# pigBond/olympics-mujoco

Hardware: AMD Instinct MI355X
Metric: env-steps/sec, 4096 UnitreeH1.walk envs per GPU, obs+reward+done+ctrl HIP kernel (higher is better)
Workload: dtype f64; 1 GPU; UnitreeH1.walk config-2: fused K1+K5 over one [T,N] block per step; T=400, envs_per_gpu=4096, launch_regime=[T,N] block per launch, io=qpos/qvel f64 + action f32 in; obs/reward/ctrl f32 + absorbing u8 out, parallelism=env-sharded x1, no data-path collective

## Files before the change

olympics-mujoco_amd/csrc/k1_il_step.hip:

```cpp
#include <cstdlib>

#include "oly_common.h"

namespace {

constexpr int THREADS = 256;
typedef unsigned int u32x4 __attribute__((ext_vector_type(4)));

template <int NQ, int NV, int NGRF, int NACT, int NU, int NOBS>
struct StaticDims {
  static constexpr int nq = NQ, nv = NV, n_grf = NGRF, n_act = NACT, nu = NU, n_obs = NOBS;
  static constexpr bool is_static = true;
  static constexpr int n_obs_ct = NOBS;
  template <int ROWS, int TH>
  static constexpr int max_chunks() {
    return (ROWS * (NQ + NV + NGRF) / 2 + ROWS * NACT / 4 + TH - 1) / TH;
  }
  __device__ explicit StaticDims(const IlDev*) {}
};
struct DynDims {
  int nq, nv, n_grf, n_act, nu, n_obs;
  static constexpr bool is_static = false;
  static constexpr int n_obs_ct = 1;
  template <int ROWS, int TH>
  static constexpr int max_chunks() { return 1; }
  __device__ explicit DynDims(const IlDev* m)
      : nq(m->nq), nv(m->nv), n_grf(m->n_grf), n_act(m->n_act), nu(m->nu), n_obs(m->n_obs) {}
};

struct IlArgs {
  const IlDev* md;
  long R;
  int N;
  const double* qpos;
  const double* qvel;
  const float* action;
  const double* grf;
  const double* prev_in;
  double* prev_out;
  void* obs;
  float* reward;
  uint8_t* absorbing;
  uint8_t* fall_code;
  void* ctrl;
  int fast;
  long tile0;
};

template <int ROWS, class D>
struct Carve {
  int q, v, g, a, tab_off, tab_str, tab_csrc, tab_act, total;
  __host__ __device__ Carve(int nq, int nv, int n_grf, int n_act, int nu, int n_obs) {
    auto al = [](int x) { return (x + 15) & ~15; };
    q = 0;
    v = q + ROWS * nq * 8;
    g = v + ROWS * nv * 8;
    a = al(g + ROWS * n_grf * 8);
    tab_off = al(a + ROWS * n_act * 4);
    tab_str = al(tab_off + n_obs * 4);
    tab_csrc = al(tab_str + n_obs * 4);
    tab_act = al(tab_csrc + nu * 4);
    total = al(tab_act + 4 * nu * 8);
  }
};

#ifndef OLY_K1_NT
#define OLY_K1_NT 1
#endif
typedef float f32x4 __attribute__((ext_vector_type(4)));
typedef double f64x2 __attribute__((ext_vector_type(2)));
__device__ __forceinline__ u32x4 ld16(const u32x4* p) {
  return (OLY_K1_NT & 1) ? __builtin_nontemporal_load(p) : *p;
}
__device__ __forceinline__ void st16(f32x4* p, f32x4 v) {
  if (OLY_K1_NT & 2) __builtin_nontemporal_store(v, p); else *p = v;
}
__device__ __forceinline__ void st16(f64x2* p, f64x2 v) {
  if (OLY_K1_NT & 2) __builtin_nontemporal_store(v, p); else *p = v;
}

#ifndef OLY_K1_ABLATE
#define OLY_K1_ABLATE 0
#endif

// ... 481 lines not shown
#pragma unroll
      for (int k = FAST_FALL - 1; k >= 0; --k)
        if (fv[k] < f_lo[k] || fv[k] > f_hi[k]) code = (unsigned)(k + 1);
      const unsigned ab = (code != 0 && use_abs) ? 1u : 0u;
      if (rt == OLY_REWARD_NONE) {
        p.reward[gr] = 0.0f;
      } else {
        if (gr < p.N) p.reward[gr] = rew_f(p.prev_in[gr]);
        if (gr + p.N < p.R)
          p.reward[gr + p.N] = rew_f(x);
        else
          p.prev_out[gr - (p.R - p.N)] = x;
      }
      unsigned a4 = 0, c4 = 0;
#pragma unroll
      for (int k = 0; k < 4; ++k) {
        const int srcl = (lane & 15) * 4 + k;
        a4 |= (unsigned)__shfl((int)ab, srcl, 64) << (8 * k);
        c4 |= (unsigned)__shfl((int)code, srcl, 64) << (8 * k);
      }
      if (lane < 16) {
        const long q4 = (row0 + (r - lane)) / 4 + lane;
        reinterpret_cast<unsigned*>(p.absorbing)[q4] = a4;
        if (p.fall_code) reinterpret_cast<unsigned*>(p.fall_code)[q4] = c4;
      }
    }

    {
      double v[NIT][OW];
#pragma unroll
      for (int it = 0; it < NIT; ++it)
#pragma unroll
        for (int k = 0; k < OW; ++k) {
          v[it][k] = sq[e_off[it][k]];
          if (NG > 0 && ((e_grf >> (it * OW + k)) & 1u)) v[it][k] = v[it][k] / 1000.0;
        }
#pragma unroll
      for (int it = 0; it < NIT; ++it) {
        const int i = tid + it * THREADS;
        if (it * THREADS + THREADS <= NOV || i < NOV) {
          if (OBS64) {
            f64x2 o;
            o.x = v[it][0]; o.y = v[it][OW - 1];
            st16(reinterpret_cast<f64x2*>(static_cast<double*>(p.obs) + row0 * NO) + i, o);
          } else {
            f32x4 o;
            o.x = (float)v[it][0]; o.y = (float)v[it][1 % OW];
            o.z = (float)v[it][2 % OW]; o.w = (float)v[it][3 % OW];
            st16(reinterpret_cast<f32x4*>(static_cast<float*>(p.obs) + row0 * NO) + i, o);
          }
        }
      }
    }

    if (with_ctrl) {
#pragma unroll
      for (int it = 0; it < NCI; ++it) {
        const int i = tid + it * THREADS;
        if (it * THREADS + THREADS <= NCV || i < NCV) {
          double u[CW];
#pragma unroll
          for (int q = 0; q < CW; ++q) {
            const int ai = c_aidx[it][q], j = c_j[it][q];
            const double a = (double)sa[ai < 0 ? 0 : ai];
            double x = a * t_act[NU + j] + t_act[j];
            const double lo = t_act[2 * NU + j], hi = t_act[3 * NU + j];
            if (x < lo) x = lo;
            if (x > hi) x = hi;
            u[q] = ai < 0 ? 0.0 : x;
          }
          if (CTRL64) {
            f64x2 o;
            o.x = u[0]; o.y = u[CW - 1];
            st16(reinterpret_cast<f64x2*>(static_cast<double*>(p.ctrl) + row0 * NU) + i, o);
          } else {
            f32x4 o;
            o.x = (float)u[0]; o.y = (float)u[1 % CW]; o.z = (float)u[2 % CW]; o.w = (float)u[3 % CW];
            st16(reinterpret_cast<f32x4*>(static_cast<float*>(p.ctrl) + row0 * NU) + i, o);
          }
        }
      }
    }
    __syncthreads();
  }
}

template <bool CTRL64>
__global__ __launch_bounds__(THREADS) void il_ctrl_kernel(const IlDev* __restrict__ md, long total,
                                                          const float* __restrict__ action,
                                                          void* __restrict__ ctrl) {
  const int nu = md->nu, n_act = md->n_act;
  const long stride = (long)gridDim.x * THREADS;
  for (long e = (long)blockIdx.x * THREADS + threadIdx.x; e < total; e += stride) {
    const long r = e / nu;
    const int j = (int)(e - r * nu);
    const int k = md->ctrl_src[j];
    double u = 0.0;
    if (k >= 0) {
      u = (double)action[r * n_act + k] * md->act_delta[k] + md->act_mean[k];
      if (u < md->ctrl_lo[k]) u = md->ctrl_lo[k];
      if (u > md->ctrl_hi[k]) u = md->ctrl_hi[k];
    }
    if (CTRL64)
      static_cast<double*>(ctrl)[e] = u;
    else
      static_cast<float*>(ctrl)[e] = (float)u;
  }
}

constexpr int DYN_ROWS = 64;

struct DynCarve {
  int a, eo, co, tact, total;
  __host__ __device__ DynCarve(int nq, int nv, int n_grf, int n_act, int nu, int n_obs) {
    auto al = [](int x) { return (x + 15) & ~15; };
    a = al(DYN_ROWS * (nq + nv + n_grf) * 8);
    eo = al(a + DYN_ROWS * n_act * 4);
    co = al(eo + DYN_ROWS * n_obs * 4);
    tact = al(co + DYN_ROWS * nu * 4);
    total = al(tact + 4 * nu * 8);
  }
};

template <bool OBS64, bool CTRL64>
__global__ __launch_bounds__(THREADS) void il_dyn_tile_kernel(IlArgs p) {
  constexpr int ROWS = DYN_ROWS;
  extern __shared__ __attribute__((aligned(16))) unsigned char lds[];
  const IlDev* __restrict__ md = p.md;
  const int nq = md->nq, nv = md->nv, n_grf = md->n_grf, n_act = md->n_act, nu = md->nu, n_obs = md->n_obs;
  const DynCarve cv(nq, nv, n_grf, n_act, nu, n_obs);
  const int tid = threadIdx.x, lane = tid & 63;
  double* sq = reinterpret_cast<double*>(lds);
  float* sa = reinterpret_cast<float*>(lds + cv.a);
  unsigned* eo = reinterpret_cast<unsigned*>(lds + cv.eo);
  int* co = reinterpret_cast<int*>(lds + cv.co);
  double* t_act = reinterpret_cast<double*>(lds + cv.tact);
  const bool with_ctrl = p.ctrl != nullptr;
  const int first_grf = n_obs - n_grf;

  auto col_off = [&](int sidx) -> int {
    if (sidx < nq) return sidx;
    if (sidx < nq + nv) return ROWS * nq + (sidx - nq);
    return ROWS * (nq + nv) + (sidx - nq - nv);
  };
  auto col_str = [&](int sidx) -> int { return sidx < nq ? nq : (sidx < nq + nv ? nv : n_grf); };

  for (int e = tid; e < ROWS * n_obs; e += THREADS) {
    const int r = e / n_obs, c = e - r * n_obs;
    const int sidx = md->src[c];
    eo[e] = (unsigned)(col_off(sidx) + r * col_str(sidx)) | (c >= first_grf && n_grf > 0 ? 0x80000000u : 0u);
  }
  for (int e = tid; e < ROWS * nu; e += THREADS) {
    const int r = e / nu, j = e - r * nu;
    const int k = md->ctrl_src[j];
    co[e] = k < 0 ? -1 : (((r * n_act + k) << 8) | j);
  }
  for (int j = tid; j < nu; j += THREADS) {
    const int k = md->ctrl_src[j];
    const int kk = k < 0 ? 0 : k;
    t_act[j] = md->act_mean[kk];
    t_act[nu + j] = md->act_delta[kk];
    t_act[2 * nu + j] = md->ctrl_lo[kk];
    t_act[3 * nu + j] = md->ctrl_hi[kk];
  }
  const int nf = md->n_fall;
  const int rt = md->reward_type;
// ... 156 lines not shown
          f64x2 o;
          o.x = u[0]; o.y = u[CW - 1];
          st16(reinterpret_cast<f64x2*>(static_cast<double*>(p.ctrl) + row0 * nu) + i, o);
        } else {
          f32x4 o;
          o.x = (float)u[0]; o.y = (float)u[1 % CW]; o.z = (float)u[2 % CW]; o.w = (float)u[3 % CW];
          st16(reinterpret_cast<f32x4*>(static_cast<float*>(p.ctrl) + row0 * nu) + i, o);
        }
      }
    }
    __syncthreads();
  }
}

using H1Dims = StaticDims<17, 17, 0, 11, 11, 32>;
using AtlasDims = StaticDims<16, 16, 0, 10, 10, 30>;
using TalosDims = StaticDims<18, 18, 0, 12, 12, 34>;
using H1FFDims = StaticDims<17, 17, 6, 11, 11, 38>;
using TalosFFDims = StaticDims<18, 18, 6, 12, 12, 40>;
using H1ArmsDims = StaticDims<25, 25, 0, 19, 19, 48>;
using H1ArmsNoBackDims = StaticDims<24, 24, 0, 18, 18, 46>;
using AtlasBackDims = StaticDims<19, 19, 0, 13, 13, 36>;
using ArmsNoBack28Dims = StaticDims<28, 28, 0, 22, 22, 54>;
using AtlasFullDims = StaticDims<31, 31, 0, 25, 25, 60>;
using TalosFullDims = StaticDims<30, 30, 0, 24, 24, 58>;

template <int ROWS, class D>
int launch_generic(oly_ctx* ctx, IlArgs a, long tile0, int out_flags, hipStream_t s) {
  const IlDev& h = ctx->il_host;
  Carve<ROWS, D> cv(h.nq, h.nv, h.n_grf, h.n_act, h.nu, h.n_obs);
  const long tiles = (a.R + ROWS - 1) / ROWS - tile0;
  if (tiles <= 0) return OLY_OK;
  if (tiles > 0x7fffffffL) OLY_FAIL(ctx, OLY_EINVAL, "oly_il_step: too many rows");
  a.tile0 = tile0;
  dim3 grid((unsigned)tiles), block(THREADS);
  const bool o64 = out_flags & OLY_OUT_OBS_F64, c64 = out_flags & OLY_OUT_CTRL_F64;
#define OLY_K1(O, C_)                                                                       \
  do {                                                                                      \
    auto k = il_step_kernel<ROWS, D, O, C_>;                                                \
    if (cv.total > 48 * 1024)                                                               \
      OLY_HIP(ctx, hipFuncSetAttribute(reinterpret_cast<const void*>(k),                    \
                                       hipFuncAttributeMaxDynamicSharedMemorySize, cv.total)); \
    hipLaunchKernelGGL(k, grid, block, cv.total, s, a);                                     \
  } while (0)
  if (o64 && c64) OLY_K1(true, true);
  else if (o64) OLY_K1(true, false);
  else if (c64) OLY_K1(false, true);
  else OLY_K1(false, false);
#undef OLY_K1
  OLY_LAUNCH_CHECK(ctx, "il_step_kernel");
  return OLY_OK;
}

template <int ROWS, class D>
int launch_fast(oly_ctx* ctx, IlArgs a, int out_flags, int wg_per_cu, hipStream_t s) {
  const long nfull = a.R / ROWS;
  if (nfull > 0) {
    const int lds = ROWS * (D::nq + D::nv + D::n_grf) * 8 + ROWS * D::n_act * 4 + 4 * D::nu * 8;
    int per_cu = (160 * 1024) / lds;
    if (per_cu > 8) per_cu = 8;
    if (wg_per_cu > 0) per_cu = wg_per_cu;
    long want = (long)ctx->num_cu * per_cu;
    if (want > nfull) want = nfull;
    IlArgs b = a;
    b.tile0 = nfull;
    dim3 grid((unsigned)want), block(THREADS);
    const bool o64 = out_flags & OLY_OUT_OBS_F64, c64 = out_flags & OLY_OUT_CTRL_F64;
#define OLY_K1T(O, C_)                                                                      \
  do {                                                                                      \
    auto k = il_tile_kernel<ROWS, D, O, C_>;                                                \
    if (lds > 48 * 1024)                                                                    \
      OLY_HIP(ctx, hipFuncSetAttribute(reinterpret_cast<const void*>(k),                    \
                                       hipFuncAttributeMaxDynamicSharedMemorySize, lds));   \
    hipLaunchKernelGGL(k, grid, block, lds, s, b);                                          \
  } while (0)
    if (o64 && c64) OLY_K1T(true, true);
    else if (o64) OLY_K1T(true, false);
    else if (c64) OLY_K1T(false, true);
    else OLY_K1T(false, false);
#undef OLY_K1T
    OLY_LAUNCH_CHECK(ctx, "il_tile_kernel");
  }
  if (nfull * ROWS < a.R) return launch_generic<ROWS, D>(ctx, a, nfull, out_flags, s);
  return OLY_OK;
}

int launch_dyn(oly_ctx* ctx, IlArgs a, int out_flags, hipStream_t s) {
  const IlDev& h = ctx->il_host;
  const DynCarve cv(h.nq, h.nv, h.n_grf, h.n_act, h.nu, h.n_obs);
  const long nfull = (a.fast && cv.total <= 150 * 1024) ? a.R / DYN_ROWS : 0;
  if (nfull > 0) {
    int per_cu = (160 * 1024) / cv.total;
    if (per_cu > 4) per_cu = 4;
    if (per_cu < 1) per_cu = 1;
    long want = (long)ctx->num_cu * per_cu;
    if (want > nfull) want = nfull;
    IlArgs b = a;
    b.tile0 = nfull;
    dim3 grid((unsigned)want), block(THREADS);
    const bool o64 = out_flags & OLY_OUT_OBS_F64, c64 = out_flags & OLY_OUT_CTRL_F64;
#define OLY_K1D(O, C_)                                                                      \
  do {                                                                                      \
    auto k = il_dyn_tile_kernel<O, C_>;                                                     \
    if (cv.total > 48 * 1024)                                                               \
      OLY_HIP(ctx, hipFuncSetAttribute(reinterpret_cast<const void*>(k),                    \
                                       hipFuncAttributeMaxDynamicSharedMemorySize, cv.total)); \
    hipLaunchKernelGGL(k, grid, block, cv.total, s, b);                                     \
  } while (0)
    if (o64 && c64) OLY_K1D(true, true);
    else if (o64) OLY_K1D(true, false);
    else if (c64) OLY_K1D(false, true);
    else OLY_K1D(false, false);
#undef OLY_K1D
    OLY_LAUNCH_CHECK(ctx, "il_dyn_tile_kernel");
  }
  if (nfull * DYN_ROWS < a.R) return launch_generic<DYN_ROWS, DynDims>(ctx, a, nfull, out_flags, s);
  return OLY_OK;
}

inline bool al16(const void* p) { return (reinterpret_cast<uintptr_t>(p) & 15) == 0; }

}

extern "C" int oly_il_configure(oly_ctx* ctx, const oly_il_model* m) {
  if (!ctx || !m) return OLY_EINVAL;
  const int n_spec = m->n_pos + m->n_vel;
  const int n_obs = n_spec - m->n_drop + m->n_grf;
  if (m->nq <= 0 || m->nv <= 0 || m->n_pos < 0 || m->n_vel < 0 || m->n_drop < 0 || m->n_grf < 0 ||
      m->n_drop > n_spec || n_obs <= 0 || n_obs > OLY_MAX_OBS || m->n_act < 0 ||
      m->n_act > OLY_MAX_ACT || m->nu < m->n_act || m->nu > OLY_MAX_ACT || m->n_fall < 0 ||
      m->n_fall > OLY_MAX_FALL)
    OLY_FAIL(ctx, OLY_EINVAL, "oly_il_configure: bad shape (n_obs=%d n_act=%d nu=%d n_fall=%d)",
             n_obs, m->n_act, m->nu, m->n_fall);
  if (!m->qpos_adr || !m->qvel_adr || (m->n_act && (!m->act_to_ctrl || !m->act_mean ||
      !m->act_delta || !m->ctrl_lo || !m->ctrl_hi)) || (m->n_fall && (!m->fall_idx || !m->fall_lo ||
      !m->fall_hi)))
    OLY_FAIL(ctx, OLY_EINVAL, "oly_il_configure: NULL table");
  ctx->il_ok = false;
  IlDev& h = ctx->il_host;
  memset(&h, 0, sizeof(h));
  h.nq = m->nq; h.nv = m->nv; h.n_pos = m->n_pos; h.n_vel = m->n_vel; h.n_drop = m->n_drop;
  h.n_grf = m->n_grf; h.n_act = m->n_act; h.nu = m->nu; h.n_obs = n_obs; h.n_fall = m->n_fall;
  h.reward_type = m->reward_type; h.reward_idx = m->reward_idx;
  h.use_absorbing = m->use_absorbing_states; h.target_velocity = m->target_velocity;
  if (h.reward_type < OLY_REWARD_NONE || h.reward_type > OLY_REWARD_X_POS)
    OLY_FAIL(ctx, OLY_EINVAL, "oly_il_configure: unknown reward_type %d", h.reward_type);
  if (h.reward_type != OLY_REWARD_NONE && (h.reward_idx < 0 || h.reward_idx >= n_obs))
    OLY_FAIL(ctx, OLY_ERANGE, "oly_il_configure: reward_idx %d outside [0,%d)", h.reward_idx, n_obs);
  for (int c = 0; c < n_obs; ++c) {
    const int slot = c + m->n_drop;
    int s;
    if (slot < m->n_pos) {
      s = m->qpos_adr[slot];
      if (s < 0 || s >= m->nq) OLY_FAIL(ctx, OLY_ERANGE, "qpos_adr[%d]=%d outside nq=%d", slot, s, m->nq);
    } else if (slot < n_spec) {
      s = m->qvel_adr[slot - m->n_pos];
      if (s < 0 || s >= m->nv) OLY_FAIL(ctx, OLY_ERANGE, "qvel_adr[%d]=%d outside nv=%d", slot - m->n_pos, s, m->nv);
      s += m->nq;
    } else {
      s = m->nq + m->nv + (slot - n_spec);
    }
    h.src[c] = (short)s;
  }
  for (int k = 0; k < m->n_fall; ++k) {
    if (m->fall_idx[k] < 0 || m->fall_idx[k] >= n_obs)
      OLY_FAIL(ctx, OLY_ERANGE, "fall_idx[%d]=%d outside [0,%d)", k, m->fall_idx[k], n_obs);
    h.fall_idx[k] = m->fall_idx[k]; h.fall_lo[k] = m->fall_lo[k]; h.fall_hi[k] = m->fall_hi[k];
    h.fall_sidx[k] = h.src[m->fall_idx[k]];
  }
  h.reward_sidx = (h.reward_type != OLY_REWARD_NONE) ? h.src[h.reward_idx] : 0;
  for (int j = 0; j < m->nu; ++j) h.ctrl_src[j] = -1;
  for (int k = 0; k < m->n_act; ++k) {
    const int j = m->act_to_ctrl[k];
    if (j < 0 || j >= m->nu) OLY_FAIL(ctx, OLY_ERANGE, "act_to_ctrl[%d]=%d outside nu=%d", k, j, m->nu);
    h.ctrl_src[j] = (short)k;
    h.act_mean[k] = m->act_mean[k]; h.act_delta[k] = m->act_delta[k];
    h.ctrl_lo[k] = m->ctrl_lo[k]; h.ctrl_hi[k] = m->ctrl_hi[k];
  }
  OLY_HIP(ctx, hipSetDevice(ctx->device));
  OLY_HIP(ctx, hipMemcpy(ctx->il_dev, &h, sizeof(h), hipMemcpyHostToDevice));
  ctx->il_ok = true;
  return OLY_OK;
}

extern "C" int oly_il_obs_dim(const oly_ctx* ctx) {
  if (!ctx || !ctx->il_ok) return OLY_ENOTCONF;
  return ctx->il_host.n_obs;
}

extern "C" int oly_il_step(oly_ctx* ctx, int T, int N, const double* qpos, const double* qvel,
                           const float* action, const double* grf_mean, const double* prev_in,
                           double* prev_out, void* obs, float* reward, uint8_t* absorbing,
                           uint8_t* fall_code, void* ctrl, int out_flags, oly_stream stream) {
  if (!ctx) return OLY_EINVAL;
  if (!ctx->il_ok) OLY_FAIL(ctx, OLY_ENOTCONF, "oly_il_step before oly_il_configure");
  const IlDev& h = ctx->il_host;
  if (T < 0 || N < 0) OLY_FAIL(ctx, OLY_EINVAL, "oly_il_step: negative T or N");
  if (T == 0 || N == 0) return OLY_OK;
  if (!qpos || !qvel || !obs || !reward || !absorbing)
    OLY_FAIL(ctx, OLY_EINVAL, "oly_il_step: NULL required pointer");
  if (h.reward_type != OLY_REWARD_NONE && (!prev_in || !prev_out))
    OLY_FAIL(ctx, OLY_EINVAL, "oly_il_step: prev_in/prev_out required by the reward");
  if (T > 1 && prev_in == prev_out && prev_in)
    OLY_FAIL(ctx, OLY_EINVAL, "oly_il_step: prev_in must not alias prev_out when T > 1");
  if (h.n_grf > 0 && !grf_mean) OLY_FAIL(ctx, OLY_EINVAL, "oly_il_step: grf_mean required (n_grf=%d)", h.n_grf);
  if (ctrl && !action) OLY_FAIL(ctx, OLY_EINVAL, "oly_il_step: ctrl requested without action");
  IlArgs a;
  a.md = ctx->il_dev; a.R = (long)T * N; a.N = N; a.qpos = qpos; a.qvel = qvel; a.action = action;
  a.grf = h.n_grf ? grf_mean : nullptr; a.prev_in = prev_in; a.prev_out = prev_out; a.obs = obs;
  a.reward = reward; a.absorbing = absorbing; a.fall_code = fall_code; a.ctrl = ctrl;
  a.fast = al16(qpos) && al16(qvel) && al16(action) && al16(grf_mean) && al16(obs) && al16(ctrl) &&
           ((reinterpret_cast<uintptr_t>(absorbing) & 3) == 0) &&
           ((reinterpret_cast<uintptr_t>(fall_code) & 3) == 0);
  a.tile0 = 0;
  auto shape = [&](int nq, int na, int no, int ng = 0) {
    return h.nq == nq && h.nv == nq && h.n_grf == ng && h.n_act == na && h.nu == na && h.n_obs == no &&
           h.n_pos == nq && h.n_vel == nq && h.n_drop == 2;
  };
  const bool fast_ok = a.fast && h.n_fall <= FAST_FALL;
  static const int wg_env = [] { const char* e = getenv("OLY_K1_WG_PER_CU"); return e ? atoi(e) : 0; }();
  static const int rows_env = [] { const char* e = getenv("OLY_K1_ROWS"); return e ? atoi(e) : 0; }();
#define OLY_K1_FAST(DIMS, DEFROWS)                                                              \
  do {                                                                                          \
    const int rows = rows_env ? rows_env : DEFROWS;                                             \
    if (rows == 64) return launch_fast<64, DIMS>(ctx, a, out_flags, wg_env, oly_s(stream));     \
    return launch_fast<128, DIMS>(ctx, a, out_flags, wg_env, oly_s(stream));                    \
  } while (0)
  if (fast_ok && shape(17, 11, 32)) OLY_K1_FAST(H1Dims, 128);
  if (fast_ok && shape(16, 10, 30)) OLY_K1_FAST(AtlasDims, 128);
  if (fast_ok && shape(18, 12, 34)) OLY_K1_FAST(TalosDims, 128);
  if (fast_ok && shape(17, 11, 38, 6)) OLY_K1_FAST(H1FFDims, 128);
  if (fast_ok && shape(18, 12, 40, 6)) OLY_K1_FAST(TalosFFDims, 128);
  if (fast_ok && shape(25, 19, 48)) OLY_K1_FAST(H1ArmsDims, 128);
  if (fast_ok && shape(24, 18, 46)) return launch_fast<128, H1ArmsNoBackDims>(ctx, a, out_flags, wg_env, oly_s(stream));
  if (fast_ok && shape(19, 13, 36)) return launch_fast<128, AtlasBackDims>(ctx, a, out_flags, wg_env, oly_s(stream));
  if (fast_ok && shape(28, 22, 54)) return launch_fast<128, ArmsNoBack28Dims>(ctx, a, out_flags, wg_env, oly_s(stream));
  if (fast_ok && shape(31, 25, 60)) return launch_fast<128, AtlasFullDims>(ctx, a, out_flags, wg_env, oly_s(stream));
  if (fast_ok && shape(30, 24, 58)) return launch_fast<128, TalosFullDims>(ctx, a, out_flags, wg_env, oly_s(stream));
#undef OLY_K1_FAST
  static const int dyn_env = [] { const char* e = getenv("OLY_K1_DYN_TILE"); return e ? atoi(e) : 1; }();
  if (dyn_env) return launch_dyn(ctx, a, out_flags, oly_s(stream));
  return launch_generic<64, DynDims>(ctx, a, 0, out_flags, oly_s(stream));
}

extern "C" int oly_il_ctrl(oly_ctx* ctx, int N, const float* action, void* ctrl, int out_flags,
                           oly_stream stream) {
  if (!ctx) return OLY_EINVAL;
  if (!ctx->il_ok) OLY_FAIL(ctx, OLY_ENOTCONF, "oly_il_ctrl before oly_il_configure");
  if (N < 0 || (N > 0 && (!action || !ctrl))) OLY_FAIL(ctx, OLY_EINVAL, "oly_il_ctrl: bad argument");
  if (N == 0) return OLY_OK;
  const long total = (long)N * ctx->il_host.nu;
  long nb = (total + THREADS - 1) / THREADS;
  if (nb > 4096) nb = 4096;
  if (out_flags & OLY_OUT_CTRL_F64)
    hipLaunchKernelGGL(il_ctrl_kernel<true>, dim3((unsigned)nb), dim3(THREADS), 0, oly_s(stream), ctx->il_dev,
                       total, action, ctrl);
  else
    hipLaunchKernelGGL(il_ctrl_kernel<false>, dim3((unsigned)nb), dim3(THREADS), 0, oly_s(stream), ctx->il_dev,
                       total, action, ctrl);
  OLY_LAUNCH_CHECK(ctx, "il_ctrl_kernel");
  return OLY_OK;
}
```

olympics-mujoco_amd/csrc/oly_api.hip:

```cpp
#include "oly_common.h"

extern "C" const char* oly_version(void) { return "olympic_hip 0.4 (gfx950)"; }
extern "C" int oly_abi_version(void) { return OLY_ABI_VERSION; }

extern "C" const char* oly_strerror(int code) {
  switch (code) {
    case OLY_OK: return "ok";
    case OLY_EINVAL: return "invalid argument";
    case OLY_ENOTCONF: return "entry point used before its configure/upload call";
    case OLY_EHIP: return "HIP runtime error";
    case OLY_ENOMEM: return "out of memory";
    case OLY_ERANGE: return "table entry out of range";
    case OLY_ENODEV: return "no usable gfx950 device";
    default: return "unknown error";
  }
}

extern "C" const char* oly_last_error(const oly_ctx* ctx) { return ctx ? ctx->err : "NULL ctx"; }

extern "C" int oly_create(oly_ctx** out, int device) {
  if (!out) return OLY_EINVAL;
  *out = nullptr;
  int count = 0;
  if (hipGetDeviceCount(&count) != hipSuccess || count <= 0) return OLY_ENODEV;
  if (device < 0) {
    if (hipGetDevice(&device) != hipSuccess) return OLY_ENODEV;
  }
  if (device >= count) return OLY_ENODEV;
  oly_ctx* ctx = new (std::nothrow) oly_ctx();
  if (!ctx) return OLY_ENOMEM;
  memset(ctx, 0, sizeof(*ctx));
  ctx->device = device;
  hipDeviceProp_t prop;
  if (hipSetDevice(device) != hipSuccess || hipGetDeviceProperties(&prop, device) != hipSuccess) {
    delete ctx;
    return OLY_ENODEV;
  }
  ctx->num_cu = prop.multiProcessorCount;
  ctx->stats_ws_bytes = sizeof(double) * OLY_STATS_MAX_BLOCKS * 2 * OLY_MAX_OBS;
  if (hipMalloc(&ctx->il_dev, sizeof(IlDev)) != hipSuccess ||
      hipMalloc(&ctx->a3_dev, sizeof(A3Dev)) != hipSuccess ||
      hipMalloc(&ctx->stats_ws, ctx->stats_ws_bytes) != hipSuccess) {
    oly_destroy(ctx);
    return OLY_ENOMEM;
  }
  *out = ctx;
  return OLY_OK;
}

extern "C" void oly_destroy(oly_ctx* ctx) {
  if (!ctx) return;
  (void)hipSetDevice(ctx->device);
  if (ctx->il_dev) (void)hipFree(ctx->il_dev);
  if (ctx->a3_dev) (void)hipFree(ctx->a3_dev);
  if (ctx->stats_ws) (void)hipFree(ctx->stats_ws);
  if (ctx->contact.geom_bodyid) (void)hipFree(ctx->contact.geom_bodyid);
  if (ctx->traj.rows) (void)hipFree(ctx->traj.rows);
  if (ctx->grf.geom_group) (void)hipFree(ctx->grf.geom_group);
  free(ctx->grf_group_host);
  delete ctx;
}

extern "C" int oly_event_create(void** ev) {
  if (!ev) return OLY_EINVAL;
  hipEvent_t e;
  if (hipEventCreate(&e) != hipSuccess) return OLY_EHIP;
  *ev = e;
  return OLY_OK;
}
extern "C" int oly_event_destroy(void* ev) {
  return hipEventDestroy(static_cast<hipEvent_t>(ev)) == hipSuccess ? OLY_OK : OLY_EHIP;
}
extern "C" int oly_event_record(void* ev, oly_stream stream) {
  return hipEventRecord(static_cast<hipEvent_t>(ev), oly_s(stream)) == hipSuccess ? OLY_OK : OLY_EHIP;
}
extern "C" int oly_event_sync(void* ev) {
  return hipEventSynchronize(static_cast<hipEvent_t>(ev)) == hipSuccess ? OLY_OK : OLY_EHIP;
}
extern "C" int oly_event_elapsed_ms(void* start, void* stop, float* ms_out) {
  if (!ms_out) return OLY_EINVAL;
  return hipEventElapsedTime(ms_out, static_cast<hipEvent_t>(start), static_cast<hipEvent_t>(stop)) ==
                 hipSuccess
             ? OLY_OK
             : OLY_EHIP;
}
extern "C" int oly_stream_sync(oly_stream stream) {
  return hipStreamSynchronize(oly_s(stream)) == hipSuccess ? OLY_OK : OLY_EHIP;
}
```

olympics-mujoco_amd/csrc/oly_common.h:

```cpp
#pragma once

#include <hip/hip_runtime.h>

#include <cstdint>
#include <cstdio>
#include <cstring>

#include "../../include/olympic_hip.h"


struct IlDev {
  int nq, nv, n_pos, n_vel, n_drop, n_grf, n_act, nu, n_obs, n_fall;
  int reward_type, reward_idx, use_absorbing, reward_sidx;
  double target_velocity;
  short src[OLY_MAX_OBS];
  int fall_idx[OLY_MAX_FALL], fall_sidx[OLY_MAX_FALL];
  double fall_lo[OLY_MAX_FALL], fall_hi[OLY_MAX_FALL];
  short ctrl_src[OLY_MAX_ACT];
  double act_mean[OLY_MAX_ACT], act_delta[OLY_MAX_ACT], ctrl_lo[OLY_MAX_ACT], ctrl_hi[OLY_MAX_ACT];
};

struct A3Dev {
  int nq, nv, nu, period, delay_frames, n_obs, pad0, pad1;
  double target_radius, mass, goal_height_ref, goal_speed_ref;
  double clock_lut[4 * OLY_MAX_PERIOD];
  double motor_offset[16], gear[16];
};

struct ContactDev {
  int ngeom, floor_body, rfoot_body, lfoot_body;
  int* geom_bodyid;
};

struct GrfDev {
  int ngeom, n_pairs;
  int pair_a[OLY_MAX_GRF_PAIRS], pair_b[OLY_MAX_GRF_PAIRS];
  int* geom_group;
};

struct TrajDev {
  int n_keys, n_traj, len, pad;
  double* rows;
};

#define OLY_STATS_MAX_BLOCKS 1024

struct oly_ctx {
  int device;
  char err[512];
  IlDev* il_dev;
  IlDev il_host;
  bool il_ok;
  A3Dev* a3_dev;
  A3Dev a3_host;
  bool a3_ok;
  ContactDev contact;
  bool contact_ok;
  TrajDev traj;
  bool traj_ok;
  GrfDev grf;
  bool grf_ok;
  int* grf_group_host;
  double* stats_ws;
  size_t stats_ws_bytes;
  bool mlp_attr_done = false;
  bool disc_attr_done = false;
  bool roll_attr_done = false;
  unsigned upd_attr_done = 0;
  unsigned scan_attr_done = 0;
  unsigned ilmlp_attr_done = 0;
  unsigned discfit_attr_done = 0;
  unsigned gail_attr_done = 0;
  int num_cu;
  unsigned ilact_attr_done = 0;
  unsigned bcfit_attr_done = 0;
  unsigned sgact_attr_done = 0;
  unsigned iqq_attr_done = 0;
  unsigned iqpi_attr_done = 0;
};

#define OLY_FAIL(ctx, code, ...)                                \
  do {                                                          \
    if (ctx) snprintf((ctx)->err, sizeof((ctx)->err), __VA_ARGS__); \
    return (code);                                              \
  } while (0)

#define OLY_HIP(ctx, expr)                                                             \
  do {                                                                                 \
    hipError_t e__ = (expr);                                                           \
    if (e__ != hipSuccess)                                                             \
      OLY_FAIL(ctx, OLY_EHIP, "%s failed: %s (%s:%d)", #expr, hipGetErrorString(e__), \
               __FILE__, __LINE__);                                                    \
  } while (0)

#define OLY_LAUNCH_CHECK(ctx, what)                                                           \
  do {                                                                                        \
    hipError_t e__ = hipGetLastError();                                                       \
    if (e__ != hipSuccess)                                                                    \
      OLY_FAIL(ctx, OLY_EHIP, "launch of %s failed: %s", what, hipGetErrorString(e__));       \
  } while (0)

int oly_stats_finish(oly_ctx* ctx, int nblocks, int64_t n, double* stats3_out, oly_stream stream);
int oly_masked_col_stats(oly_ctx* ctx, long B, int Dx, int D, const float* x, const int32_t* mask, double* colstats,
                         int accumulate, double* copy_out, oly_stream stream);
int oly_a3_step_strided(oly_ctx* ctx, int N, const oly_a3_inputs* in, const oly_a3_state* st, void* obs, float* rew6,
                        float* reward, uint8_t* done, int out_flags, int compact_base, oly_stream stream);

static inline hipStream_t oly_s(oly_stream s) { return reinterpret_cast<hipStream_t>(s); }

__device__ __forceinline__ double wave_sum(double v) {
#pragma unroll
  for (int off = 32; off > 0; off >>= 1) v += __shfl_down(v, off, 64);
  return v;
}
```

Measured before the change: 11.99 billion env-steps/s.

## Add small-tile one-launch row kernel with precomputed per-tile gather tables

Adds a new K1 step kernel that handles a small tile of rows (16 by default) per block and launches one block per tile, replacing the persistent large-tile kernel for row counts up to a threshold. A per-tile gather table of obs source offsets, ctrl source indices, fall/reward offsets and actuator constants is built on the host at configure time and uploaded once. This drops per-element index math inside the kernel and gives many more small blocks to hide latency on this small T*N workload. In exchange it costs extra table loads per block, a larger grid, and more configure-time work.

```diff
diff --git a/olympics-mujoco_amd/csrc/k1_il_step.hip b/olympics-mujoco_amd/csrc/k1_il_step.hip
--- a/olympics-mujoco_amd/csrc/k1_il_step.hip
+++ b/olympics-mujoco_amd/csrc/k1_il_step.hip
@@ -1,5 +1,8 @@
 #include <cstdlib>
-
+#include <memory>
+#include <new>
+
+#include "k1_step_tab.h"
 #include "oly_common.h"
 
 namespace {
@@ -647,6 +650,286 @@
       }
     }
     __syncthreads();
+  }
+}
+
+#ifndef OLY_K1_STEP_ROWS
+#define OLY_K1_STEP_ROWS 16
+#endif
+#ifndef OLY_K1_STEP_THREADS
+#define OLY_K1_STEP_THREADS 256
+#endif
+constexpr int STEP_ROWS = OLY_K1_STEP_ROWS, STEP_THREADS = OLY_K1_STEP_THREADS;
+#ifndef OLY_K1_STEP_MAX_ROWS
+#define OLY_K1_STEP_MAX_ROWS 262144
+#endif
+constexpr long STEP_MAX_ROWS = OLY_K1_STEP_MAX_ROWS;
+static_assert(STEP_ROWS <= OLY_K1_STEP_ROWS_MAX && FAST_FALL == OLY_K1_STEP_FALL, "IlStepTab is sized for these");
+typedef unsigned int u32x2 __attribute__((ext_vector_type(2)));
+
+struct IlStepArgs : IlArgs {
+  const IlStepTab* tab;
+};
+
+template <int ROWS, int TH, class D, bool OBS64, bool CTRL64>
+__global__ __launch_bounds__(TH) void il_row_kernel(IlStepArgs p) {
+  static_assert(D::is_static, "step kernel needs compile-time dimensions");
+  static_assert(ROWS % 4 == 0 && ROWS <= 64 && TH % 64 == 0, "tile shape");
+  constexpr int NQ = D::nq, NV = D::nv, NG = D::n_grf, NA = D::n_act, NU = D::nu, NO = D::n_obs;
+  constexpr int CQ = ROWS * NQ / 2, CV = ROWS * NV / 2, CG = ROWS * NG / 2, CA = ROWS * NA / 4;
+  constexpr int KQ = (CQ + TH - 1) / TH, KV = (CV + TH - 1) / TH, KG = (CG + TH - 1) / TH, KA = (CA + TH - 1) / TH;
+  constexpr int ND = NQ + NV + NG;
+  constexpr int OW = OBS64 ? 2 : 4, NOV = ROWS * NO / OW, NIT = (NOV + TH - 1) / TH;
+  constexpr int CW = CTRL64 ? 2 : 4, NCV = ROWS * NU / CW, NCI = (NCV + TH - 1) / TH;
+  static_assert(2 * NU <= TH, "the actuator constants are staged by one 16-B load per lane");
+
+  __shared__ __attribute__((aligned(16))) unsigned char lds[ROWS * ND * 8 + ROWS * NA * 4 + 4 * NU * 8];
+  double* sq = reinterpret_cast<double*>(lds);
+  double* sv = sq + ROWS * NQ;
+  double* sg = sv + ROWS * NV;
+  float* sa = reinterpret_cast<float*>(lds + (size_t)ROWS * ND * 8);
+  double* t_act = reinterpret_cast<double*>(lds + (size_t)ROWS * ND * 8 + (size_t)ROWS * NA * 4);
+  const IlDev* __restrict__ md = p.md;
+  const IlStepTab* __restrict__ tb = p.tab;
+  const int tid = threadIdx.x, lane = tid & 63;
+  const bool with_ctrl = p.ctrl != nullptr;
+  const long row0 = (long)blockIdx.x * ROWS;
+  const int rows = (p.R - row0 < ROWS) ? (int)(p.R - row0) : ROWS;
+  const bool full = rows == ROWS;
+
+  u32x4 rq[KQ], rv[KV], rg[KG > 0 ? KG : 1], ra[KA];
+  if (full) {
+    const u32x4* gq = reinterpret_cast<const u32x4*>(p.qpos + row0 * NQ) + tid;
+    const u32x4* gv = reinterpret_cast<const u32x4*>(p.qvel + row0 * NV) + tid;
+#pragma unroll
+    for (int k = 0; k < KQ; ++k)
+      if (k * TH + TH <= CQ || tid + k * TH < CQ) rq[k] = ld16(gq + k * TH);
+#pragma unroll
+    for (int k = 0; k < KV; ++k)
+      if (k * TH + TH <= CV || tid + k * TH < CV) rv[k] = ld16(gv + k * TH);
+    if (NG > 0) {
+      const u32x4* gg = reinterpret_cast<const u32x4*>(p.grf + row0 * NG) + tid;
+#pragma unroll
+      for (int k = 0; k < KG; ++k)
+        if (k * TH + TH <= CG || tid + k * TH < CG) rg[k] = ld16(gg + k * TH);
+    }
+    if (with_ctrl) {
+      const u32x4* ga = reinterpret_cast<const u32x4*>(p.action + row0 * NA) + tid;
+#pragma unroll
+      for (int k = 0; k < KA; ++k)
+        if (k * TH + TH <= CA || tid + k * TH < CA) ra[k] = ld16(ga + k * TH);
+    }
+  }
+
+  unsigned eo[NIT][OW];
+  int co[NCI][CW];
+  if (full) {
+#pragma unroll
+    for (int it = 0; it < NIT; ++it) {
+      const int i = tid + it * TH;
+      const bool in = it * TH + TH <= NOV || i < NOV;
+      if constexpr (OBS64) {
+        const u32x2 t = in ? reinterpret_cast<const u32x2*>(tb->obs)[i] : u32x2{0u, 0u};
+        eo[it][0] = t.x; eo[it][1] = t.y;
+      } else {
+        const u32x4 t = in ? reinterpret_cast<const u32x4*>(tb->obs)[i] : u32x4{0u, 0u, 0u, 0u};
+        eo[it][0] = t.x; eo[it][1] = t.y; eo[it][2] = t.z; eo[it][3] = t.w;
+      }
+    }
+    if (with_ctrl) {
+#pragma unroll
+      for (int it = 0; it < NCI; ++it) {
+        const int i = tid + it * TH;
+        const bool in = it * TH + TH <= NCV || i < NCV;
+        if constexpr (CTRL64) {
+          const u32x2 t = in ? reinterpret_cast<const u32x2*>(tb->ctl)[i] : u32x2{0u, 0u};
+          co[it][0] = (int)t.x; co[it][1] = (int)t.y;
+        } else {
+          const u32x4 t = in ? reinterpret_cast<const u32x4*>(tb->ctl)[i] : u32x4{0u, 0u, 0u, 0u};
+          co[it][0] = (int)t.x; co[it][1] = (int)t.y; co[it][2] = (int)t.z; co[it][3] = (int)t.w;
+        }
+      }
+    }
+  }
+  u32x4 ta = {0u, 0u, 0u, 0u};
+  if (with_ctrl && tid < 2 * NU) ta = reinterpret_cast<const u32x4*>(tb->t_act)[tid];
+  int f_off[FAST_FALL], f_str[FAST_FALL];
+  double f_lo[FAST_FALL], f_hi[FAST_FALL];
+#pragma unroll
+  for (int k = 0; k < FAST_FALL; ++k) {
+    f_off[k] = tb->f_off[k]; f_str[k] = tb->f_str[k];
+    f_lo[k] = tb->f_lo[k]; f_hi[k] = tb->f_hi[k];
+  }
+  const unsigned f_grf = (unsigned)tb->f_grf;
+  const int rew_off = tb->rew_off, rew_str = tb->rew_str;
+  const bool rew_grf = tb->rew_grf != 0;
+  const int rt = md->reward_type;
+  const double tvel = md->target_velocity;
+  const int use_abs = md->use_absorbing;
+  auto rew_f = [&](double s) -> float {
+    if (rt == OLY_REWARD_TARGET_VELOCITY) {
+      const double dv = s - tvel;
+      return (float)exp(-(dv * dv));
+    }
+    return (float)s;
+  };
+  const int r = tid - (TH - 64);
+  const long gr = row0 + r;
+  double prev0 = 0.0;
+  if (r >= 0 && r < rows && rt != OLY_REWARD_NONE && gr < p.N) prev0 = p.prev_in[gr];
+
+  if (full) {
+    u32x4* lq = reinterpret_cast<u32x4*>(sq) + tid;
+    u32x4* lv = reinterpret_cast<u32x4*>(sv) + tid;
+    u32x4* la = reinterpret_cast<u32x4*>(sa) + tid;
+#pragma unroll
+    for (int k = 0; k < KQ; ++k)
+      if (k * TH + TH <= CQ || tid + k * TH < CQ) lq[k * TH] = rq[k];
+#pragma unroll
+    for (int k = 0; k < KV; ++k)
+      if (k * TH + TH <= CV || tid + k * TH < CV) lv[k * TH] = rv[k];
+    if (NG > 0) {
+      u32x4* lg = reinterpret_cast<u32x4*>(sg) + tid;
+#pragma unroll
+      for (int k = 0; k < KG; ++k)
+        if (k * TH + TH <= CG || tid + k * TH < CG) lg[k * TH] = rg[k];
+    }
+    if (with_ctrl) {
+#pragma unroll
+      for (int k = 0; k < KA; ++k)
+        if (k * TH + TH <= CA || tid + k * TH < CA) la[k * TH] = ra[k];
+    }
+  } else {
+    for (int i = tid; i < rows * NQ; i += TH) sq[i] = p.qpos[row0 * NQ + i];
+    for (int i = tid; i < rows * NV; i += TH) sv[i] = p.qvel[row0 * NV + i];
+    if (NG > 0)
+      for (int i = tid; i < rows * NG; i += TH) sg[i] = p.grf[row0 * NG + i];
+    if (with_ctrl)
+      for (int i = tid; i < rows * NA; i += TH) sa[i] = p.action[row0 * NA + i];
+  }
+  if (with_ctrl && tid < 2 * NU) reinterpret_cast<u32x4*>(t_act)[tid] = ta;
+  __syncthreads();
+
+  if (r >= 0 && r < ROWS) {
+    const bool live = r < rows;
+    double fv[FAST_FALL];
+#pragma unroll
+    for (int k = 0; k < FAST_FALL; ++k) {
+      fv[k] = sq[f_off[k] + r * f_str[k]];
+      if (NG > 0 && ((f_grf >> k) & 1u)) fv[k] = fv[k] / 1000.0;
+    }
+    double x = sq[rew_off + r * rew_str];
+    if (NG > 0 && rew_grf) x = x / 1000.0;
+    unsigned code = 0;
+#pragma unroll
+    for (int k = FAST_FALL - 1; k >= 0; --k)
+      if (fv[k] < f_lo[k] || fv[k] > f_hi[k]) code = (unsigned)(k + 1);
+    const unsigned ab = (code != 0 && use_abs) ? 1u : 0u;
+    if (live) {
+      if (rt == OLY_REWARD_NONE) {
+        p.reward[gr] = 0.0f;
+      } else {
+        if (gr < p.N) p.reward[gr] = rew_f(prev0);
+        if (gr + p.N < p.R)
+          p.reward[gr + p.N] = rew_f(x);
+        else
+          p.prev_out[gr - (p.R - p.N)] = x;
+      }
+    }
+    if (full) {
+      unsigned a4 = 0, c4 = 0;
+#pragma unroll
+      for (int k = 0; k < 4; ++k) {
+        const int srcl = (lane & (ROWS / 4 - 1)) * 4 + k;
+        a4 |= (unsigned)__shfl((int)ab, srcl, 64) << (8 * k);
+        c4 |= (unsigned)__shfl((int)code, srcl, 64) << (8 * k);
+      }
+      if (lane < ROWS / 4) {
+        const long q4 = row0 / 4 + lane;
+        reinterpret_cast<unsigned*>(p.absorbing)[q4] = a4;
+        if (p.fall_code) reinterpret_cast<unsigned*>(p.fall_code)[q4] = c4;
+      }
+    } else if (live) {
+      p.absorbing[gr] = (uint8_t)ab;
+      if (p.fall_code) p.fall_code[gr] = (uint8_t)code;
+    }
+  }
+
+  if (full) {
+    double v[NIT][OW];
+#pragma unroll
+    for (int it = 0; it < NIT; ++it)
+#pragma unroll
+      for (int k = 0; k < OW; ++k) {
+        v[it][k] = sq[eo[it][k] & 0x7fffffffu];
+        if (NG > 0 && (eo[it][k] >> 31)) v[it][k] = v[it][k] / 1000.0;
+      }
+#pragma unroll
+    for (int it = 0; it < NIT; ++it) {
+      const int i = tid + it * TH;
+      if (it * TH + TH <= NOV || i < NOV) {
+        if (OBS64) {
+          f64x2 o;
+          o.x = v[it][0]; o.y = v[it][OW - 1];
+          st16(reinterpret_cast<f64x2*>(static_cast<double*>(p.obs) + row0 * NO) + i, o);
+        } else {
+          f32x4 o;
+          o.x = (float)v[it][0]; o.y = (float)v[it][1 % OW];
+          o.z = (float)v[it][2 % OW]; o.w = (float)v[it][3 % OW];
+          st16(reinterpret_cast<f32x4*>(static_cast<float*>(p.obs) + row0 * NO) + i, o);
+        }
+      }
+    }
+  } else {
+    for (int e = tid; e < rows * NO; e += TH) {
+      const unsigned o = tb->obs[e];
+      double v = sq[o & 0x7fffffffu];
+      if (NG > 0 && (o >> 31)) v = v / 1000.0;
+      if (OBS64)
+        static_cast<double*>(p.obs)[row0 * NO + e] = v;
+      else
+        static_cast<float*>(p.obs)[row0 * NO + e] = (float)v;
+    }
+  }
+
+  if (with_ctrl) {
+    auto ctrl_val = [&](int c) -> double {
+      const int j = c < 0 ? 0 : (c & 0xff), ai = c >> 8;
+      const double a = (double)sa[c < 0 ? 0 : ai];
+      double x = a * t_act[NU + j] + t_act[j];
+      const double lo = t_act[2 * NU + j], hi = t_act[3 * NU + j];
+      if (x < lo) x = lo;
+      if (x > hi) x = hi;
+      return c < 0 ? 0.0 : x;
+    };
+    if (full) {
+#pragma unroll
+      for (int it = 0; it < NCI; ++it) {
+        const int i = tid + it * TH;
+        if (it * TH + TH <= NCV || i < NCV) {
+          double u[CW];
+#pragma unroll
+          for (int q = 0; q < CW; ++q) u[q] = ctrl_val(co[it][q]);
+          if (CTRL64) {
+            f64x2 o;
+            o.x = u[0]; o.y = u[CW - 1];
+            st16(reinterpret_cast<f64x2*>(static_cast<double*>(p.ctrl) + row0 * NU) + i, o);
+          } else {
+            f32x4 o;
+            o.x = (float)u[0]; o.y = (float)u[1 % CW]; o.z = (float)u[2 % CW]; o.w = (float)u[3 % CW];
+            st16(reinterpret_cast<f32x4*>(static_cast<float*>(p.ctrl) + row0 * NU) + i, o);
+          }
+        }
+      }
+    } else {
+      for (int e = tid; e < rows * NU; e += TH) {
+        const double u = ctrl_val(tb->ctl[e]);
+        if (CTRL64)
+          static_cast<double*>(p.ctrl)[row0 * NU + e] = u;
+        else
+          static_cast<float*>(p.ctrl)[row0 * NU + e] = (float)u;
+      }
+    }
   }
 }
 
@@ -969,6 +1252,23 @@
     OLY_LAUNCH_CHECK(ctx, "il_tile_kernel");
   }
   if (nfull * ROWS < a.R) return launch_generic<ROWS, D>(ctx, a, nfull, out_flags, s);
+  return OLY_OK;
+}
+
+template <class D>
+int launch_step(oly_ctx* ctx, const IlArgs& a, int out_flags, hipStream_t s) {
+  const long tiles = (a.R + STEP_ROWS - 1) / STEP_ROWS;
+  if (tiles > 0x7fffffffL) OLY_FAIL(ctx, OLY_EINVAL, "oly_il_step: too many rows");
+  IlStepArgs b;
+  static_cast<IlArgs&>(b) = a;
+  b.tab = ctx->il_step_dev;
+  dim3 grid((unsigned)tiles), block(STEP_THREADS);
+  const bool o64 = out_flags & OLY_OUT_OBS_F64, c64 = out_flags & OLY_OUT_CTRL_F64;
+  if (o64 && c64) hipLaunchKernelGGL((il_row_kernel<STEP_ROWS, STEP_THREADS, D, true, true>), grid, block, 0, s, b);
+  else if (o64) hipLaunchKernelGGL((il_row_kernel<STEP_ROWS, STEP_THREADS, D, true, false>), grid, block, 0, s, b);
+  else if (c64) hipLaunchKernelGGL((il_row_kernel<STEP_ROWS, STEP_THREADS, D, false, true>), grid, block, 0, s, b);
+  else hipLaunchKernelGGL((il_row_kernel<STEP_ROWS, STEP_THREADS, D, false, false>), grid, block, 0, s, b);
+  OLY_LAUNCH_CHECK(ctx, "il_row_kernel");
   return OLY_OK;
 }
 
@@ -1066,6 +1366,10 @@
   }
   OLY_HIP(ctx, hipSetDevice(ctx->device));
   OLY_HIP(ctx, hipMemcpy(ctx->il_dev, &h, sizeof(h), hipMemcpyHostToDevice));
+  std::unique_ptr<IlStepTab> tab(new (std::nothrow) IlStepTab);
+  if (!tab) OLY_FAIL(ctx, OLY_ENOMEM, "oly_il_configure: out of host memory");
+  oly_k1_step_tab_build(h, STEP_ROWS, tab.get());
+  OLY_HIP(ctx, hipMemcpy(ctx->il_step_dev, tab.get(), sizeof(IlStepTab), hipMemcpyHostToDevice));
   ctx->il_ok = true;
   return OLY_OK;
 }
@@ -1107,8 +1411,13 @@
   const bool fast_ok = a.fast && h.n_fall <= FAST_FALL;
   static const int wg_env = [] { const char* e = getenv("OLY_K1_WG_PER_CU"); return e ? atoi(e) : 0; }();
   static const int rows_env = [] { const char* e = getenv("OLY_K1_ROWS"); return e ? atoi(e) : 0; }();
+  static const int step_env = [] { const char* e = getenv("OLY_K1_STEP"); return e ? atoi(e) : -1; }();
+  const bool step_side = step_env >= 0 ? step_env != 0 : (!rows_env && a.R <= STEP_MAX_ROWS);
+#define OLY_K1_STEP_SIDE(DIMS) \
+  if (step_side) return launch_step<DIMS>(ctx, a, out_flags, oly_s(stream))
 #define OLY_K1_FAST(DIMS, DEFROWS)                                                              \
   do {                                                                                          \
+    OLY_K1_STEP_SIDE(DIMS);                                                                     \
     const int rows = rows_env ? rows_env : DEFROWS;                                             \
     if (rows == 64) return launch_fast<64, DIMS>(ctx, a, out_flags, wg_env, oly_s(stream));     \
     return launch_fast<128, DIMS>(ctx, a, out_flags, wg_env, oly_s(stream));                    \
@@ -1119,12 +1428,18 @@
   if (fast_ok && shape(17, 11, 38, 6)) OLY_K1_FAST(H1FFDims, 128);
   if (fast_ok && shape(18, 12, 40, 6)) OLY_K1_FAST(TalosFFDims, 128);
   if (fast_ok && shape(25, 19, 48)) OLY_K1_FAST(H1ArmsDims, 128);
+  if (fast_ok && shape(24, 18, 46)) OLY_K1_STEP_SIDE(H1ArmsNoBackDims);
   if (fast_ok && shape(24, 18, 46)) return launch_fast<128, H1ArmsNoBackDims>(ctx, a, out_flags, wg_env, oly_s(stream));
+  if (fast_ok && shape(19, 13, 36)) OLY_K1_STEP_SIDE(AtlasBackDims);
   if (fast_ok && shape(19, 13, 36)) return launch_fast<128, AtlasBackDims>(ctx, a, out_flags, wg_env, oly_s(stream));
+  if (fast_ok && shape(28, 22, 54)) OLY_K1_STEP_SIDE(ArmsNoBack28Dims);
   if (fast_ok && shape(28, 22, 54)) return launch_fast<128, ArmsNoBack28Dims>(ctx, a, out_flags, wg_env, oly_s(stream));
+  if (fast_ok && shape(31, 25, 60)) OLY_K1_STEP_SIDE(AtlasFullDims);
   if (fast_ok && shape(31, 25, 60)) return launch_fast<128, AtlasFullDims>(ctx, a, out_flags, wg_env, oly_s(stream));
+  if (fast_ok && shape(30, 24, 58)) OLY_K1_STEP_SIDE(TalosFullDims);
   if (fast_ok && shape(30, 24, 58)) return launch_fast<128, TalosFullDims>(ctx, a, out_flags, wg_env, oly_s(stream));
 #undef OLY_K1_FAST
+#undef OLY_K1_STEP_SIDE
   static const int dyn_env = [] { const char* e = getenv("OLY_K1_DYN_TILE"); return e ? atoi(e) : 1; }();
   if (dyn_env) return launch_dyn(ctx, a, out_flags, oly_s(stream));
   return launch_generic<64, DynDims>(ctx, a, 0, out_flags, oly_s(stream));
diff --git a/olympics-mujoco_amd/csrc/k1_step_tab.h b/olympics-mujoco_amd/csrc/k1_step_tab.h
--- /dev/null
+++ b/olympics-mujoco_amd/csrc/k1_step_tab.h
@@ -0,0 +1,43 @@
+#pragma once
+
+#include "oly_common.h"
+
+inline void oly_k1_step_tab_build(const IlDev& h, int rows, IlStepTab* t) {
+  memset(t, 0, sizeof(*t));
+  t->rows = rows;
+  auto col_off = [&](int sidx) -> int {
+    return sidx < h.nq ? sidx : sidx < h.nq + h.nv ? rows * h.nq + (sidx - h.nq) : rows * (h.nq + h.nv) + (sidx - h.nq - h.nv);
+  };
+  auto col_str = [&](int sidx) -> int { return sidx < h.nq ? h.nq : sidx < h.nq + h.nv ? h.nv : h.n_grf; };
+  auto is_grf = [&](int sidx) -> bool { return h.n_grf > 0 && sidx >= h.nq + h.nv; };
+  for (int k = 0; k < OLY_K1_STEP_FALL; ++k) {
+    const int kk = k < h.n_fall ? k : 0;
+    const int sidx = h.fall_sidx[kk];
+    t->f_off[k] = col_off(sidx);
+    t->f_str[k] = col_str(sidx);
+    if (is_grf(sidx)) t->f_grf |= 1 << k;
+    t->f_lo[k] = k < h.n_fall ? h.fall_lo[kk] : -__builtin_huge_val();
+    t->f_hi[k] = k < h.n_fall ? h.fall_hi[kk] : __builtin_huge_val();
+  }
+  t->rew_off = col_off(h.reward_sidx);
+  t->rew_str = col_str(h.reward_sidx);
+  t->rew_grf = is_grf(h.reward_sidx) ? 1 : 0;
+  for (int j = 0; j < h.nu; ++j) {
+    const int k = h.ctrl_src[j];
+    const int kk = k < 0 ? 0 : k;
+    t->t_act[j] = h.act_mean[kk];
+    t->t_act[h.nu + j] = h.act_delta[kk];
+    t->t_act[2 * h.nu + j] = h.ctrl_lo[kk];
+    t->t_act[3 * h.nu + j] = h.ctrl_hi[kk];
+  }
+  for (int r = 0; r < rows; ++r) {
+    for (int c = 0; c < h.n_obs; ++c) {
+      const int sidx = h.src[c];
+      t->obs[r * h.n_obs + c] = (unsigned)(col_off(sidx) + r * col_str(sidx)) | (is_grf(sidx) ? 0x80000000u : 0u);
+    }
+    for (int j = 0; j < h.nu; ++j) {
+      const int k = h.ctrl_src[j];
+      t->ctl[r * h.nu + j] = k < 0 ? -1 : (((r * h.n_act + k) << 8) | j);
+    }
+  }
+}
diff --git a/olympics-mujoco_amd/csrc/oly_api.hip b/olympics-mujoco_amd/csrc/oly_api.hip
--- a/olympics-mujoco_amd/csrc/oly_api.hip
+++ b/olympics-mujoco_amd/csrc/oly_api.hip
@@ -39,6 +39,7 @@
   ctx->num_cu = prop.multiProcessorCount;
   ctx->stats_ws_bytes = sizeof(double) * OLY_STATS_MAX_BLOCKS * 2 * OLY_MAX_OBS;
   if (hipMalloc(&ctx->il_dev, sizeof(IlDev)) != hipSuccess ||
+      hipMalloc(&ctx->il_step_dev, sizeof(IlStepTab)) != hipSuccess ||
       hipMalloc(&ctx->a3_dev, sizeof(A3Dev)) != hipSuccess ||
       hipMalloc(&ctx->stats_ws, ctx->stats_ws_bytes) != hipSuccess) {
     oly_destroy(ctx);
@@ -52,6 +53,7 @@
   if (!ctx) return;
   (void)hipSetDevice(ctx->device);
   if (ctx->il_dev) (void)hipFree(ctx->il_dev);
+  if (ctx->il_step_dev) (void)hipFree(ctx->il_step_dev);
   if (ctx->a3_dev) (void)hipFree(ctx->a3_dev);
   if (ctx->stats_ws) (void)hipFree(ctx->stats_ws);
   if (ctx->contact.geom_bodyid) (void)hipFree(ctx->contact.geom_bodyid);
diff --git a/olympics-mujoco_amd/csrc/oly_common.h b/olympics-mujoco_amd/csrc/oly_common.h
--- a/olympics-mujoco_amd/csrc/oly_common.h
+++ b/olympics-mujoco_amd/csrc/oly_common.h
@@ -2,6 +2,7 @@
 
 #include <hip/hip_runtime.h>
 
+#include <cstddef>
 #include <cstdint>
 #include <cstdio>
 #include <cstring>
@@ -19,6 +20,20 @@
   short ctrl_src[OLY_MAX_ACT];
   double act_mean[OLY_MAX_ACT], act_delta[OLY_MAX_ACT], ctrl_lo[OLY_MAX_ACT], ctrl_hi[OLY_MAX_ACT];
 };
+
+#define OLY_K1_STEP_ROWS_MAX 32
+#define OLY_K1_STEP_FALL 8
+struct IlStepTab {
+  int f_off[OLY_K1_STEP_FALL], f_str[OLY_K1_STEP_FALL];
+  double f_lo[OLY_K1_STEP_FALL], f_hi[OLY_K1_STEP_FALL];
+  int f_grf, rew_off, rew_str, rew_grf;
+  int rows, pad[3];
+  double t_act[4 * OLY_MAX_ACT];
+  unsigned obs[OLY_K1_STEP_ROWS_MAX * OLY_MAX_OBS];
+  int ctl[OLY_K1_STEP_ROWS_MAX * OLY_MAX_ACT];
+};
+static_assert(offsetof(IlStepTab, t_act) % 16 == 0 && offsetof(IlStepTab, obs) % 16 == 0 &&
+              offsetof(IlStepTab, ctl) % 16 == 0, "the lanes read their entries with 16-byte loads");
 
 struct A3Dev {
   int nq, nv, nu, period, delay_frames, n_obs, pad0, pad1;
@@ -51,6 +66,7 @@
   IlDev* il_dev;
   IlDev il_host;
   bool il_ok;
+  IlStepTab* il_step_dev;
   A3Dev* a3_dev;
   A3Dev a3_host;
   bool a3_ok;
```

After: 12.05 billion env-steps/s (median of 2 runs). No clear change (+0.5%).
